# vainglorygame/analyzer

Measured on AMD Instinct MI355X. Metric: matches/sec rated (whole node), 3v3 TrueSkill, 1M-player roster, higher is better.
Workload: dtype fp32; 1 GPU; global_batch=10000000, seq_len=6, players=1000000, matches_per_gpu=10000000, team_size=3, parallelism=dp1, mode=exact, bench_config=2, skew=1, force_merge=False

## Files before the change

analyzer_amd/csrc/radix_sort.hip:

```cpp
#include <hip/hip_runtime.h>

#include <cstdlib>

#include "common.h"
#include "kernels.h"

namespace ana {

namespace {

#ifndef ANA_SORT_THREADS
#define ANA_SORT_THREADS 512
#endif
constexpr int kThreads = ANA_SORT_THREADS;
constexpr int kWaves = kThreads / 64;
constexpr int kItems = 16;
constexpr int kTile = kThreads * kItems;
constexpr int kRadix = 256;
constexpr int kRadixMax = 1024;

__device__ __forceinline__ int64_t xcd_tile(int64_t tiles) {
  const int64_t i = blockIdx.x, q = tiles >> 3, r = tiles & 7, x = i & 7;
  return x * q + (x < r ? x : r) + (i >> 3);
}

template <int NT>
__device__ __forceinline__ uint32_t ld32(const uint32_t* p) {
  if constexpr (NT >= 1) return __builtin_nontemporal_load(p);
  else return *p;
}
template <int NT>
__device__ __forceinline__ void st32(uint32_t* p, uint32_t v) {
  if constexpr (NT == 1) __builtin_nontemporal_store(v, p);
  else *p = v;
}

__device__ __forceinline__ uint32_t block_exclusive_scan(uint32_t x, uint32_t* wsum,
                                                         uint32_t* total) {
  const int lane = threadIdx.x & 63, wv = threadIdx.x >> 6;
  uint32_t inc = x;
#pragma unroll
  for (int off = 1; off < 64; off <<= 1) {
    const uint32_t y = __shfl_up(inc, off);
    if (lane >= off) inc += y;
  }
  if (lane == 63) wsum[wv] = inc;
  __syncthreads();
  uint32_t before = 0, all = 0;
#pragma unroll
  for (int w = 0; w < kWaves; ++w) {
    if (w < wv) before += wsum[w];
    all += wsum[w];
  }
  if (total) *total = all;
  __syncthreads();
  return before + inc - x;
}

template <int KS>
__device__ __forceinline__ void decode_tile_keys(const int32_t* __restrict__ rec, uint32_t kend,
                                                 int64_t base, int64_t n, uint32_t* lk, uint32_t knone) {
  constexpr int S = 2 * KS, R = S + 2;
  const uint32_t lo = (uint32_t)base;
  const uint32_t hi = (uint32_t)(base + kTile < n ? base + kTile : n);
  const uint32_t m_lo = lo / S, m_hi = (hi + S - 1) / S;
  for (uint32_t m = m_lo + threadIdx.x; m < m_hi; m += kThreads) {
    const int32_t* src = rec + (int64_t)m * R;
    int32_t r[R];
    if constexpr (R % 4 == 0) {
#pragma unroll
      for (int k = 0; k < R / 4; ++k) {
        const int4 v = reinterpret_cast<const int4*>(src)[k];
        r[4 * k] = v.x; r[4 * k + 1] = v.y; r[4 * k + 2] = v.z; r[4 * k + 3] = v.w;
      }
    } else {
#pragma unroll
      for (int k = 0; k < R; ++k) r[k] = src[k];
    }
    const bool rates = early_status<KS>(r, (int64_t)kend) == kRated;
    const uint32_t m0 = (uint32_t)r[S];
#pragma unroll
    for (int j = 0; j < S; ++j) {
      const uint32_t slot = m * S + j;
      const int pos = j < KS ? j : j - KS;
      const bool in_roster = pos < (j < KS ? meta_n0(m0) : meta_n1(m0));
      if (slot >= lo && slot < hi) lk[slot - lo] = rates && in_roster ? (uint32_t)r[j] : knone;
    }
  }
}

struct SchedInit {
  int32_t* deps = nullptr;
  uint32_t* ctrl = nullptr;
  int nz = 0;
  int32_t* epoch_bump = nullptr;
};

template <int KS, int RB = 8, int NT = 0>
__global__ void __launch_bounds__(kThreads)
radix_upsweep(const uint32_t* __restrict__ keys, const int32_t* __restrict__ rec, uint32_t kend,
              int64_t n, int shift, uint32_t* __restrict__ counts, int64_t tiles, SchedInit init = {},
              uint32_t knone = 0u) {
  constexpr int kR = 1 << RB;
  __shared__ uint32_t hist[kWaves][kR];
  __shared__ uint32_t lkeys[KS > 0 ? kTile : 1];
  const int tid = threadIdx.x, wv = tid >> 6;
  for (int i = tid; i < kWaves * kR; i += kThreads) (&hist[0][0])[i] = 0u;
  const int64_t tile = xcd_tile(tiles);
  const int64_t base = tile * kTile;
  if constexpr (KS > 0) {
    if (init.deps) {
      constexpr int S = 2 * KS;
      const int64_t hi = base + kTile < n ? base + kTile : n;
      for (int64_t m = (base + S - 1) / S + tid; m < (hi + S - 1) / S; m += kThreads) init.deps[m] = 0;
    }
    if (blockIdx.x == 0) {
      if (tid < init.nz) init.ctrl[tid] = 0u;
      if (tid == 0 && init.epoch_bump) init.epoch_bump[0] += 1;
    }
  }
  if constexpr (KS > 0) decode_tile_keys<KS>(rec, kend, base, n, lkeys, knone ? knone : kend);
  __syncthreads();
#pragma unroll
  for (int k = 0; k < kItems; ++k) {
    const int64_t idx = base + k * kThreads + tid;
    if (idx < n) {
      const uint32_t key = KS > 0 ? lkeys[k * kThreads + tid] : ld32<NT>(keys + idx);
      atomicAdd(&hist[wv][(key >> shift) & (kR - 1)], 1u);
    }
  }
  __syncthreads();
#pragma unroll
  for (int d = tid; d < kR; d += kThreads) {
    uint32_t c = 0;
#pragma unroll
    for (int w = 0; w < kWaves; ++w) c += hist[w][d];
    counts[(int64_t)d * tiles + tile] = c;
  }
}

template <int DPT>
__device__ __forceinline__ void digits_exclusive_scan(uint32_t (&v)[DPT], uint32_t* wsum,
                                                      uint32_t* total) {
  uint32_t s = 0;
#pragma unroll
  for (int j = 0; j < DPT; ++j) {
    const uint32_t x = v[j];
    v[j] = s;
    s += x;
  }
  const uint32_t before = block_exclusive_scan(s, wsum, total);
#pragma unroll
  for (int j = 0; j < DPT; ++j) v[j] += before;
}

__global__ void __launch_bounds__(kThreads)
radix_rowscan(uint32_t* __restrict__ counts, int64_t tiles, uint32_t* __restrict__ totals) {
  __shared__ uint32_t wsum[kWaves];
  constexpr int kPer = 4;
  uint32_t* row = counts + (int64_t)blockIdx.x * tiles;
  uint32_t carry = 0;
  for (int64_t start = 0; start < tiles; start += kThreads * kPer) {
    uint32_t v[kPer], s = 0;
#pragma unroll
    for (int q = 0; q < kPer; ++q) {
      const int64_t t = start + (int64_t)threadIdx.x * kPer + q;
      v[q] = t < tiles ? row[t] : 0u;
      s += v[q];
    }
    uint32_t all;
    uint32_t ex = carry + block_exclusive_scan(s, wsum, &all);
#pragma unroll
    for (int q = 0; q < kPer; ++q) {
      const int64_t t = start + (int64_t)threadIdx.x * kPer + q;
      if (t < tiles) row[t] = ex;
      ex += v[q];
    }
    carry += all;
  }
  if (threadIdx.x == 0) totals[blockIdx.x] = carry;
}

struct RunEnds {
  uint32_t kf, vf, kl, vl;
};
constexpr uint32_t kRunEmpty = 0xffffffffu;

template <int KS, bool LINK, int RB = 8, int NT = 0>
__global__ void __launch_bounds__(kThreads)
radix_downsweep(const uint32_t* __restrict__ kin, const uint32_t* __restrict__ vin,
                const int32_t* __restrict__ rec, uint32_t kend,
                uint32_t* __restrict__ kout, uint32_t* __restrict__ vout, int64_t n, int shift,
                const uint32_t* __restrict__ counts, const uint32_t* __restrict__ totals,
                int64_t tiles, int slots_per_match, uint32_t* __restrict__ link,
                uint32_t vlo = 0u, uint32_t vhi = 0xffffffffu, int bounds = 1,
                RunEnds* __restrict__ bnd = nullptr, int nd = 0, uint32_t knone = 0u) {
  constexpr int kR = 1 << RB;
  constexpr int DPT = kR >= kThreads ? kR / kThreads : 1;
  static_assert(kR % kThreads == 0 || kThreads % kR == 0, "radix and block must divide");
  __shared__ uint32_t skey[kTile];
  __shared__ uint32_t sval[kTile];
  __shared__ uint32_t wcnt[kWaves][kR];
  __shared__ uint32_t tstart[kR];
  __shared__ uint32_t gstart[kR];
  __shared__ uint32_t wsum[kWaves];
  const int tid = threadIdx.x, lane = tid & 63, wv = tid >> 6;
  const int64_t tile = xcd_tile(tiles);
  const int64_t base = tile * kTile;
  for (int i = tid; i < kWaves * kR; i += kThreads) (&wcnt[0][0])[i] = 0u;
  const bool local_ends = LINK && bnd != nullptr;
  if (!local_ends) {
    uint32_t v[DPT];
#pragma unroll
    for (int j = 0; j < DPT; ++j) v[j] = tid * DPT + j < kR ? totals[tid * DPT + j] : 0u;
    digits_exclusive_scan<DPT>(v, wsum, nullptr);
#pragma unroll
    for (int j = 0; j < DPT; ++j)
      if (tid * DPT + j < kR) gstart[tid * DPT + j] = v[j] + counts[(int64_t)(tid * DPT + j) * tiles + tile];
  }
  if constexpr (KS > 0)
    decode_tile_keys<KS>(rec, kend, base, n, sval, knone ? knone : kend);
  __syncthreads();

  const uint64_t lt_mask = (1ull << lane) - 1ull;
  uint32_t key[kItems], val[kItems], rank[kItems];
#pragma unroll
  for (int it = 0; it < kItems; ++it) {
    const int64_t idx = base + (int64_t)(wv * kItems + it) * 64 + lane;
    const bool valid = idx < n;
    if constexpr (KS > 0) key[it] = valid ? sval[(wv * kItems + it) * 64 + lane] : 0xffffffffu;
    else key[it] = valid ? ld32<NT>(kin + idx) : 0xffffffffu;
    if constexpr (KS == 0) val[it] = valid ? ld32<NT>(vin + idx) : 0u;
    else val[it] = (uint32_t)idx;
  }
#pragma unroll
  for (int it = 0; it < kItems; ++it) {
    const uint32_t d = (key[it] >> shift) & (kR - 1);
    uint64_t peers = ~0ull;
#pragma unroll
    for (int b = 0; b < RB; ++b) {
      const uint64_t bal = __ballot((d >> b) & 1u);
      peers &= ((d >> b) & 1u) ? bal : ~bal;
    }
    const uint32_t before = (uint32_t)__popcll(peers & lt_mask);
    const uint32_t run = wcnt[wv][d];
    rank[it] = run + before;
    if (before == (uint32_t)__popcll(peers) - 1u) wcnt[wv][d] = run + (uint32_t)__popcll(peers);
  }
  __syncthreads();
  {
    uint32_t v[DPT];
#pragma unroll
    for (int j = 0; j < DPT; ++j) {
      const int d = tid * DPT + j;
      uint32_t s = 0;
      if (d < kR) {
#pragma unroll
        for (int w = 0; w < kWaves; ++w) {
          const uint32_t c = wcnt[w][d];
          wcnt[w][d] = s;
          s += c;
        }
      }
      v[j] = s;
    }
    digits_exclusive_scan<DPT>(v, wsum, nullptr);
#pragma unroll
    for (int j = 0; j < DPT; ++j)
      if (tid * DPT + j < kR) tstart[tid * DPT + j] = v[j];
  }
  __syncthreads();
#pragma unroll
  for (int it = 0; it < kItems; ++it) {
    const uint32_t d = (key[it] >> shift) & (kR - 1);
    const uint32_t pos = tstart[d] + wcnt[wv][d] + rank[it];
    skey[pos] = key[it];
    sval[pos] = val[it];
  }
  __syncthreads();
  const int64_t nvalid = n - base < kTile ? n - base : kTile;
  if constexpr (LINK) {
    if (local_ends && bounds && tid < nd) {
      const uint32_t e = tid + 1 < kR ? tstart[tid + 1] : (uint32_t)kTile;
      if (tstart[tid] == e) bnd[tile * nd + tid].kf = kRunEmpty;
    }
  }
#pragma unroll
  for (int k = 0; k < kItems; ++k) {
    const int i = k * kThreads + tid;
    if (i < nvalid) {
      const uint32_t kk = skey[i];
      const uint32_t d = (kk >> shift) & (kR - 1);
      const int64_t o = local_ends ? 0 : (int64_t)gstart[d] + (i - (int64_t)tstart[d]);
      if constexpr (!LINK) {
        st32<NT>(kout + o, kk);
        st32<NT>(vout + o, sval[i]);
      } else {
        const int hi = d + 1 < (uint32_t)kR ? (int)tstart[d + 1] : kTile;
        const bool first = i == (int)tstart[d];
        const bool last = i + 1 == hi || i + 1 >= nvalid;
        const uint32_t v = sval[i];
        if (bounds && (first || last)) {
          if (local_ends) {
            if ((int)d < nd) {
              RunEnds* r = bnd + tile * nd + d;
              if (first) { r->kf = kk; r->vf = v; }
              if (last) { r->kl = kk; r->vl = v; }
            }
          } else {
            st32<NT>(kout + o, kk);
            st32<NT>(vout + o, v);
          }
        }
        if (kk < kend && v >= vlo && v < vhi) {
          uint32_t w = (!last && skey[i + 1] == kk) ? sval[i + 1] / (uint32_t)slots_per_match
                                                     : kNoMatch;
          if (!first && skey[i - 1] == kk) w |= kLinkHasPred;
          st32<NT>(link + v, w);
        }
      }
    }
  }
}

static bool local_runs() {
  const char* e = getenv("ANA_SCHED_RUNS");
  return !(e && atoi(e) == 0);
}

static int link_parts(int64_t n) {
  if (const char* e = getenv("ANA_LINK_PARTS")) {
    const int v = atoi(e);
    if (v >= 1) return v > 16 ? 16 : v;
  }
  const int64_t bytes = n * 4, part = 256ll << 20;
  return (int)((bytes + part - 1) / part);
}

template <int RB = 8>
__global__ void __launch_bounds__(kThreads)
sched_fixup(const uint32_t* __restrict__ kout, const uint32_t* __restrict__ vout, int64_t n,
            uint32_t kend, const uint32_t* __restrict__ counts, const uint32_t* __restrict__ totals,
            int64_t tiles, int slots_per_match, uint32_t* __restrict__ link) {
  constexpr int kR = 1 << RB;
  __shared__ uint32_t wsum[kWaves];
  const int d = blockIdx.y;
  const uint32_t tot = totals[d];
  if (tot == 0) return;
  uint32_t below = 0;
#pragma unroll
  for (int j = threadIdx.x; j < kR; j += kThreads) below += j < d ? totals[j] : 0u;
  uint32_t all = 0;
  const uint32_t before = block_exclusive_scan(below, wsum, &all);
  (void)before;
  const uint32_t dstart = all;
  const int64_t t = (int64_t)blockIdx.x * kThreads + threadIdx.x;
  if (t >= tiles) return;
  const uint32_t* row = counts + (int64_t)d * tiles;
  const uint32_t c0 = row[t];
  const uint32_t c1 = t + 1 < tiles ? row[t + 1] : tot;
  if (c1 == c0) return;
  const int64_t of = (int64_t)dstart + c0, ol = (int64_t)dstart + c1 - 1;
  const uint32_t kf = kout[of], kl = kout[ol];
  const bool pred = kf < kend && of > 0 && kout[of - 1] == kf;
  const bool succ = kl < kend && ol + 1 < n && kout[ol + 1] == kl;
  const uint32_t nxt = succ ? vout[ol + 1] / (uint32_t)slots_per_match : kNoMatch;
  if (of == ol) {
    if (kf < kend) link[vout[of]] = nxt | (pred ? kLinkHasPred : 0u);
    return;
  }
  if (pred) {
    const uint32_t v = vout[of];
    link[v] |= kLinkHasPred;
  }
  if (succ) {
    const uint32_t v = vout[ol];
    link[v] = (link[v] & ~kMatchMask) | nxt;
  }
}

constexpr int kRunsMaxDigits = 32;

__global__ void __launch_bounds__(kThreads)
sched_runs_last(const RunEnds* __restrict__ bnd, int64_t tiles, int nd, int32_t* __restrict__ seglast) {
  __shared__ int32_t wmax[kWaves];
  const int d = blockIdx.y;
  const int64_t t = (int64_t)blockIdx.x * kThreads + threadIdx.x;
  int32_t x = (t < tiles && bnd[t * nd + d].kf != kRunEmpty) ? (int32_t)t : -1;
#pragma unroll
  for (int off = 32; off >= 1; off >>= 1) x = max(x, __shfl_xor(x, off));
  if ((threadIdx.x & 63) == 0) wmax[threadIdx.x >> 6] = x;
  __syncthreads();
  if (threadIdx.x == 0) {
    int32_t m = wmax[0];
#pragma unroll
    for (int w = 1; w < kWaves; ++w) m = max(m, wmax[w]);
    seglast[(int64_t)d * gridDim.x + blockIdx.x] = m;
  }
}

__global__ void __launch_bounds__(kThreads)
sched_runs_fixup(const RunEnds* __restrict__ bnd, int64_t tiles, int nd, const int32_t* __restrict__ seglast,
                 uint32_t kend, int slots_per_match, uint32_t* __restrict__ link) {
  __shared__ int32_t wmax[kWaves];
  __shared__ int32_t carry_s;
  const int d = blockIdx.y, lane = threadIdx.x & 63, wv = threadIdx.x >> 6;
  const int64_t seg = blockIdx.x;
  if (wv == 0) {
    int32_t c = -1;
    for (int64_t q = lane; q < seg; q += 64) c = max(c, seglast[(int64_t)d * gridDim.x + q]);
#pragma unroll
    for (int off = 32; off >= 1; off >>= 1) c = max(c, __shfl_xor(c, off));
    if (lane == 0) carry_s = c;
  }
  const int64_t t = seg * kThreads + threadIdx.x;
  RunEnds me = {kRunEmpty, 0u, kRunEmpty, 0u};
  if (t < tiles) me = bnd[t * nd + d];
  const bool full = me.kf != kRunEmpty;
  int32_t x = full ? (int32_t)t : -1;
#pragma unroll
  for (int off = 1; off < 64; off <<= 1) {
    const int32_t y = __shfl_up(x, off);
    if (lane >= off) x = max(x, y);
  }
  if (lane == 63) wmax[wv] = x;
  __syncthreads();
  int32_t before = carry_s;
  for (int w = 0; w < wv; ++w) before = max(before, wmax[w]);
  int32_t ex = __shfl_up(x, 1);
  ex = lane == 0 ? -1 : ex;
  const int32_t pred = max(before, ex);
  if (!full || pred < 0 || me.kf >= kend) return;
  const RunEnds pr = bnd[(int64_t)pred * nd + d];
  if (pr.kl != me.kf) return;
  atomicOr(&link[me.vf], kLinkHasPred);
  atomicAnd(&link[pr.vl], ~kMatchMask | (me.vf / (uint32_t)slots_per_match));
}

constexpr int kChainLowBits = 12;
constexpr int kChainRB = 6;
constexpr uint32_t kChainEmpty = 0xffffffffu;
constexpr bool kChainDefault = true;

__device__ __forceinline__ void chain_sort_round(const uint32_t (&key)[kItems], const uint32_t (&val)[kItems],
                                                 int shift, uint32_t* skey, uint32_t* sval,
                                                 uint32_t (*wcnt)[1 << kChainRB], uint32_t* tstart,
                                                 uint32_t* wsum) {
  constexpr int kR = 1 << kChainRB;
  static_assert(kR <= kThreads, "one digit per thread in the scan");
  const int tid = threadIdx.x, lane = tid & 63, wv = tid >> 6;
  const uint64_t lt_mask = (1ull << lane) - 1ull;
  for (int i = tid; i < kWaves * kR; i += kThreads) (&wcnt[0][0])[i] = 0u;
  __syncthreads();
  uint32_t rank[kItems];
#pragma unroll
  for (int it = 0; it < kItems; ++it) {
    const uint32_t d = (key[it] >> shift) & (kR - 1);
    uint64_t peers = ~0ull;
#pragma unroll
    for (int b = 0; b < kChainRB; ++b) {
      const uint64_t bal = __ballot((d >> b) & 1u);
      peers &= ((d >> b) & 1u) ? bal : ~bal;
    }
    const uint32_t before = (uint32_t)__popcll(peers & lt_mask);
    const uint32_t run = wcnt[wv][d];
    rank[it] = run + before;
    if (before == (uint32_t)__popcll(peers) - 1u) wcnt[wv][d] = run + (uint32_t)__popcll(peers);
  }
  __syncthreads();
  {
    uint32_t v[1];
    uint32_t s = 0;
    if (tid < kR) {
#pragma unroll
      for (int w = 0; w < kWaves; ++w) {
        const uint32_t c = wcnt[w][tid];
        wcnt[w][tid] = s;
        s += c;
      }
    }
    v[0] = s;
    digits_exclusive_scan<1>(v, wsum, nullptr);
    if (tid < kR) tstart[tid] = v[0];
  }
  __syncthreads();
#pragma unroll
  for (int it = 0; it < kItems; ++it) {
    const uint32_t d = (key[it] >> shift) & (kR - 1);
    const uint32_t pos = tstart[d] + wcnt[wv][d] + rank[it];
    skey[pos] = key[it];
    sval[pos] = val[it];
  }
  __syncthreads();
}

template <int KS, int NT>
__global__ void __launch_bounds__(kThreads)
sched_chain(const uint32_t* __restrict__ kin, const uint32_t* __restrict__ vin,
            const int32_t* __restrict__ rec, uint32_t kend, int64_t n, int low,
            const uint32_t* __restrict__ totals, int slots_per_match, uint32_t* __restrict__ link,
            uint32_t vlo, uint32_t vhi, int64_t matches, SchedInit init) {
  constexpr int kR = 1 << kChainRB;
  __shared__ uint32_t skey[kTile];
  __shared__ uint32_t sval[kTile];
  __shared__ uint32_t last_seen[1 << kChainLowBits];
  __shared__ uint32_t wcnt[kWaves][kR];
  __shared__ uint32_t tstart[kR];
  __shared__ uint32_t wsum[kWaves];
  const int tid = threadIdx.x, lane = tid & 63, wv = tid >> 6;
  const uint32_t lmask = (1u << low) - 1u;
  for (int e = tid; e <= (int)lmask; e += kThreads) last_seen[e] = kChainEmpty;
  int64_t start = 0, cnt = n;
  if constexpr (KS > 0) {
    if (init.deps)
      for (int64_t m = tid; m < matches; m += kThreads) init.deps[m] = 0;
    if (tid < init.nz) init.ctrl[tid] = 0u;
    if (tid == 0 && init.epoch_bump) init.epoch_bump[0] += 1;
  } else {
    uint32_t below = 0;
    const uint32_t x = tid < (int)blockIdx.x ? totals[tid] : 0u;
    block_exclusive_scan(x, wsum, &below);
    start = below;
    cnt = totals[blockIdx.x];
  }
  for (int64_t base = 0; base < cnt; base += kTile) {
    const int64_t nvalid = cnt - base < kTile ? cnt - base : kTile;
    uint32_t key[kItems], val[kItems];
    if constexpr (KS > 0) {
      decode_tile_keys<KS>(rec, kend, base, n, sval, kend);
      __syncthreads();
    }
#pragma unroll
    for (int it = 0; it < kItems; ++it) {
      const int p = (wv * kItems + it) * 64 + lane;
      const bool valid = p < nvalid;
      const int64_t idx = start + base + p;
      if constexpr (KS > 0) {
        key[it] = valid ? sval[p] : 0xffffffffu;
        val[it] = (uint32_t)idx;
      } else {
        key[it] = valid ? ld32<NT>(kin + idx) : 0xffffffffu;
        val[it] = valid ? ld32<NT>(vin + idx) : 0u;
      }
    }
    chain_sort_round(key, val, 0, skey, sval, wcnt, tstart, wsum);
    if (low > kChainRB) {
#pragma unroll
      for (int it = 0; it < kItems; ++it) {
        const int p = (wv * kItems + it) * 64 + lane;
        key[it] = skey[p];
        val[it] = sval[p];
      }
      chain_sort_round(key, val, kChainRB, skey, sval, wcnt, tstart, wsum);
    }
    uint32_t is_last = 0u, has = 0u;
#pragma unroll 2
    for (int k = 0; k < kItems; ++k) {
      const int i = k * kThreads + tid;
      if (i < nvalid) {
        const uint32_t kk = skey[i];
        if (kk < kend) {
          const uint32_t v = sval[i];
          const bool next = i + 1 < nvalid && skey[i + 1] == kk;
          bool pred = i > 0 && skey[i - 1] == kk;
          if (!pred) {
            const uint32_t t = last_seen[kk & lmask];
            if (t != kChainEmpty) {
              pred = true;
              const uint32_t ts = t & kMatchMask;
              if (ts >= vlo && ts < vhi) link[ts] = v / (uint32_t)slots_per_match | (t & kLinkHasPred);
            }
          }
          if (next) {
            if (v >= vlo && v < vhi)
              link[v] = sval[i + 1] / (uint32_t)slots_per_match | (pred ? kLinkHasPred : 0u);
          } else {
            is_last |= 1u << k;
          }
          if (pred) has |= 1u << k;
        }
      }
    }
    __syncthreads();
#pragma unroll 2
    for (int k = 0; k < kItems; ++k) {
      const int i = k * kThreads + tid;
      if (is_last >> k & 1u) last_seen[skey[i] & lmask] = sval[i] | (has >> k & 1u ? kLinkHasPred : 0u);
    }
    __syncthreads();
  }
  __syncthreads();
  for (int e = tid; e <= (int)lmask; e += kThreads) {
    const uint32_t t = last_seen[e];
    if (t != kChainEmpty) {
      const uint32_t ts = t & kMatchMask;
      if (ts >= vlo && ts < vhi) link[ts] = kNoMatch | (t & kLinkHasPred);
    }
  }
}

}

size_t radix_sort_workspace_bytes(int64_t n) {
  const int64_t tiles = (n + kTile - 1) / kTile;
  return (size_t)(tiles * kRadixMax + kRadixMax) * 4;
}

int launch_radix_sort_pairs(uint32_t* keys, uint32_t* vals, uint32_t* keys_alt, uint32_t* vals_alt,
                            int64_t n, int bits, void* ws, int* result_in_alt, hipStream_t s) {
  *result_in_alt = 0;
  if (n <= 0) return 0;
  if (n > 0x7fffffffLL || bits < 1 || bits > 32) return (int)hipErrorInvalidValue;
  const int64_t tiles = (n + kTile - 1) / kTile;
  uint32_t* counts = static_cast<uint32_t*>(ws);
  uint32_t* totals = counts + tiles * kRadix;
  uint32_t *ki = keys, *vi = vals, *ko = keys_alt, *vo = vals_alt;
  for (int shift = 0; shift < bits; shift += 8) {
    hipLaunchKernelGGL(radix_upsweep<0>, dim3((unsigned)tiles), dim3(kThreads), 0, s, ki, nullptr,
                       0u, n, shift, counts, tiles);
    hipLaunchKernelGGL(radix_rowscan, dim3(kRadix), dim3(kThreads), 0, s, counts, tiles, totals);
    hipLaunchKernelGGL((radix_downsweep<0, false>), dim3((unsigned)tiles), dim3(kThreads), 0, s, ki,
                       vi, nullptr, 0u, ko, vo, n, shift, counts, totals, tiles, 1, nullptr);
    std::swap(ki, ko);
    std::swap(vi, vo);
    *result_in_alt ^= 1;
  }
  return (int)hipGetLastError();
}

template <int K, int RB, int NT>
static void sched_sort_k(const int32_t* rec, int64_t n, uint32_t kend, int bits, uint32_t* ka,
                         uint32_t* va, uint32_t* kb, uint32_t* vb, uint32_t* counts,
                         int64_t tiles, uint32_t* link, const SchedInit& init, bool chain,
                         hipStream_t s) {
  constexpr int S = 2 * K;
  constexpr int kR = 1 << RB;
  uint32_t* totals = counts + tiles * kR;
  const dim3 grid((unsigned)tiles), block(kThreads);
  const uint32_t *ki = nullptr, *vi = nullptr;
  uint32_t *ko = kb, *vo = vb;
  if (chain) {
    const int low = bits < kChainLowBits ? bits : kChainLowBits, top = bits - low;
    const int parts = link_parts(n);
    if (top > 0) {
      const uint32_t nb = ((kend - 1u) >> low) + 1u;
      const uint32_t knone = nb < (uint32_t)kR ? nb << low : kend;
      hipLaunchKernelGGL((radix_upsweep<K, RB, NT>), grid, block, 0, s, nullptr, rec, kend, n, low, counts, tiles,
                         init, knone);
      hipLaunchKernelGGL(radix_rowscan, dim3(kR), block, 0, s, counts, tiles, totals);
      hipLaunchKernelGGL((radix_downsweep<K, false, RB, NT>), grid, block, 0, s, nullptr, nullptr, rec, kend, ko,
                         vo, n, low, counts, totals, tiles, S, nullptr, 0u, 0xffffffffu, 1, nullptr, 0, knone);
      for (int q = 0; q < parts; ++q)
        hipLaunchKernelGGL((sched_chain<0, NT>), dim3(nb), block, 0, s, ko, vo, nullptr, kend, n, low,
                           totals, S, link, (uint32_t)(n * q / parts), (uint32_t)(n * (q + 1) / parts),
                           n / S, SchedInit{});
    } else {
      for (int q = 0; q < parts; ++q)
        hipLaunchKernelGGL((sched_chain<K, NT>), dim3(1), block, 0, s, nullptr, nullptr, rec, kend, n, low,
                           nullptr, S, link, (uint32_t)(n * q / parts), (uint32_t)(n * (q + 1) / parts),
                           n / S, q == 0 ? init : SchedInit{});
    }
    return;
  }
  for (int shift = 0; shift < bits; shift += RB) {
    const bool first = shift == 0, last = shift + RB >= bits;
    const int nd = bits - shift < RB ? 1 << (bits - shift) : kR;
    if (last && !first && nd <= kRunsMaxDigits && local_runs()) {
      RunEnds* bnd = reinterpret_cast<RunEnds*>(counts);
      const int64_t nseg = (tiles + kThreads - 1) / kThreads;
      int32_t* seglast = reinterpret_cast<int32_t*>(bnd + tiles * nd);
      const int parts = link_parts(n);
      for (int q = 0; q < parts; ++q)
        hipLaunchKernelGGL((radix_downsweep<0, true, RB, NT>), grid, block, 0, s, ki, vi, nullptr, kend, ko, vo,
                           n, shift, counts, totals, tiles, S, link, (uint32_t)(n * q / parts),
                           (uint32_t)(n * (q + 1) / parts), q == 0 ? 1 : 0, bnd, nd);
      const dim3 sgrid((unsigned)nseg, (unsigned)nd);
      hipLaunchKernelGGL(sched_runs_last, sgrid, block, 0, s, bnd, tiles, nd, seglast);
      hipLaunchKernelGGL(sched_runs_fixup, sgrid, block, 0, s, bnd, tiles, nd, seglast, kend, S, link);
      break;
    }
    if (first)
      hipLaunchKernelGGL((radix_upsweep<K, RB, NT>), grid, block, 0, s, nullptr, rec, kend, n, shift, counts, tiles,
                         init);
    else
      hipLaunchKernelGGL((radix_upsweep<0, RB, NT>), grid, block, 0, s, ki, nullptr, kend, n, shift, counts, tiles);
    hipLaunchKernelGGL(radix_rowscan, dim3(kR), block, 0, s, counts, tiles, totals);
    const int parts = last ? link_parts(n) : 1;
    if (first && last)
      for (int q = 0; q < parts; ++q)
        hipLaunchKernelGGL((radix_downsweep<K, true, RB, NT>), grid, block, 0, s, nullptr, nullptr, rec, kend, ko,
                           vo, n, shift, counts, totals, tiles, S, link, (uint32_t)(n * q / parts),
                           (uint32_t)(n * (q + 1) / parts), q == 0 ? 1 : 0);
    else if (first)
      hipLaunchKernelGGL((radix_downsweep<K, false, RB, NT>), grid, block, 0, s, nullptr, nullptr, rec, kend, ko,
                         vo, n, shift, counts, totals, tiles, S, nullptr);
    else if (last)
      for (int q = 0; q < parts; ++q)
        hipLaunchKernelGGL((radix_downsweep<0, true, RB, NT>), grid, block, 0, s, ki, vi, nullptr, kend, ko, vo,
                           n, shift, counts, totals, tiles, S, link, (uint32_t)(n * q / parts),
                           (uint32_t)(n * (q + 1) / parts), q == 0 ? 1 : 0);
    else
      hipLaunchKernelGGL((radix_downsweep<0, false, RB, NT>), grid, block, 0, s, ki, vi, nullptr, kend, ko, vo, n,
                         shift, counts, totals, tiles, S, nullptr);
    if (last)
      hipLaunchKernelGGL((sched_fixup<RB>), dim3((unsigned)((tiles + kThreads - 1) / kThreads), kR), block,
                         0, s, ko, vo, n, kend, counts, totals, tiles, S, link);
    ki = ko;
    vi = vo;
    ko = ko == kb ? ka : kb;
    vo = vo == vb ? va : vb;
  }
}

int launch_sched_sort(int K, const int32_t* rec, int64_t M, uint32_t num_players, uint32_t* ka,
                      uint32_t* va, uint32_t* kb, uint32_t* vb, void* ws, uint32_t* link,
                      hipStream_t s, int32_t* deps, uint32_t* ctrl, int nz, int32_t* epoch_bump,
                      int sort_nt) {
  const int64_t n = M * 2 * K;
  if (n <= 0) return 0;
  if (n > kMaxSlots) return (int)hipErrorInvalidValue;
  int bits = 1;
  while (bits < 32 && (1ull << bits) <= (uint64_t)num_players) ++bits;
  const int64_t tiles = (n + kTile - 1) / kTile;
  uint32_t* counts = static_cast<uint32_t*>(ws);
  SchedInit init;
  init.deps = deps;
  init.ctrl = ctrl;
  init.nz = ctrl ? nz : 0;
  init.epoch_bump = epoch_bump;
  const char* rb_e = getenv("ANA_SORT_RB");
  const char* nt_e = getenv("ANA_SORT_NT");
  const int rb_env = rb_e ? atoi(rb_e) : 8;
  const int nt = nt_e ? atoi(nt_e) : sort_nt >= 0 ? sort_nt : 0;
  const bool wide = bits <= 20 && rb_env == 10;
  const char* chain_e = getenv("ANA_SCHED_CHAIN");
  const int top = bits > kChainLowBits ? bits - kChainLowBits : 0;
  const bool chain_pays = (n >> top) <= 2 * kTile + n / 128;
  const bool chain = (chain_e ? atoi(chain_e) != 0 : kChainDefault && chain_pays) && bits <= 20 && !wide &&
                     local_runs();
  const bool known = with_team_size(K, [&](auto k) {
    constexpr int kK = decltype(k)::value;
    if (wide) sched_sort_k<kK, 10, 0>(rec, n, num_players, bits, ka, va, kb, vb, counts, tiles, link, init, chain, s);
    else if (nt == 1) sched_sort_k<kK, 8, 1>(rec, n, num_players, bits, ka, va, kb, vb, counts, tiles, link, init, chain, s);
    else if (nt == 2) sched_sort_k<kK, 8, 2>(rec, n, num_players, bits, ka, va, kb, vb, counts, tiles, link, init, chain, s);
    else sched_sort_k<kK, 8, 0>(rec, n, num_players, bits, ka, va, kb, vb, counts, tiles, link, init, chain, s);
  });
  return known ? (int)hipGetLastError() : (int)hipErrorInvalidValue;
}

}
```

Baseline: 1.578 billion matches/s.

## Write chain links in partitioned order then scatter back with an unpartition kernel

When the key space spans several buckets, the chain kernel no longer writes links by random match index across multiple partition passes. It instead writes each link into the partitioned key buffer in bucket order, buffering the current tile in shared memory and deferring tile tails. A new unpartition kernel then scatters those links back to original positions one tile at a time and uses vectorized stores where it can. The aim is to replace scattered global writes and the repeated link_parts launches with coalesced writes, at the cost of an extra kernel pass, extra reads of the partitioned buffers, and more shared memory per block.

New measurement: 1.680 billion matches/s, median of 6. 6.4% higher.

```diff
diff --git a/analyzer_amd/csrc/radix_sort.hip b/analyzer_amd/csrc/radix_sort.hip
--- a/analyzer_amd/csrc/radix_sort.hip
+++ b/analyzer_amd/csrc/radix_sort.hip
@@ -442,6 +442,7 @@
 constexpr uint32_t kChainEmpty = 0xffffffffu;
 constexpr bool kChainDefault = true;
 
+template <bool VALS = true>
 __device__ __forceinline__ void chain_sort_round(const uint32_t (&key)[kItems], const uint32_t (&val)[kItems],
                                                  int shift, uint32_t* skey, uint32_t* sval,
                                                  uint32_t (*wcnt)[1 << kChainRB], uint32_t* tstart,
@@ -489,20 +490,25 @@
     const uint32_t d = (key[it] >> shift) & (kR - 1);
     const uint32_t pos = tstart[d] + wcnt[wv][d] + rank[it];
     skey[pos] = key[it];
-    sval[pos] = val[it];
-  }
-  __syncthreads();
-}
-
-template <int KS, int NT>
+    if constexpr (VALS) sval[pos] = val[it];
+  }
+  __syncthreads();
+}
+
+constexpr uint32_t kLinkDeferred = 0xfffffffeu;
+constexpr uint32_t kLinkSkip = 0xffffffffu;
+
+template <int KS, int NT, bool LINES>
 __global__ void __launch_bounds__(kThreads)
-sched_chain(const uint32_t* __restrict__ kin, const uint32_t* __restrict__ vin,
+sched_chain(uint32_t* kio, const uint32_t* __restrict__ vin,
             const int32_t* __restrict__ rec, uint32_t kend, int64_t n, int low,
             const uint32_t* __restrict__ totals, int slots_per_match, uint32_t* __restrict__ link,
             uint32_t vlo, uint32_t vhi, int64_t matches, SchedInit init) {
   constexpr int kR = 1 << kChainRB;
+  static_assert(!LINES || KS == 0, "bucket positions need the partition");
   __shared__ uint32_t skey[kTile];
   __shared__ uint32_t sval[kTile];
+  __shared__ uint32_t lbuf[LINES ? kTile : 1];
   __shared__ uint32_t last_seen[1 << kChainLowBits];
   __shared__ uint32_t wcnt[kWaves][kR];
   __shared__ uint32_t tstart[kR];
@@ -523,6 +529,7 @@
     start = below;
     cnt = totals[blockIdx.x];
   }
+  const uint32_t kbase = LINES ? (uint32_t)blockIdx.x << low : 0u;
   for (int64_t base = 0; base < cnt; base += kTile) {
     const int64_t nvalid = cnt - base < kTile ? cnt - base : kTile;
     uint32_t key[kItems], val[kItems];
@@ -538,63 +545,201 @@
       if constexpr (KS > 0) {
         key[it] = valid ? sval[p] : 0xffffffffu;
         val[it] = (uint32_t)idx;
+      } else if constexpr (!LINES) {
+        key[it] = valid ? ld32<NT>(kio + idx) : 0xffffffffu;
+        val[it] = valid ? ld32<NT>(vin + idx) : 0u;
       } else {
-        key[it] = valid ? ld32<NT>(kin + idx) : 0xffffffffu;
-        val[it] = valid ? ld32<NT>(vin + idx) : 0u;
-      }
-    }
-    chain_sort_round(key, val, 0, skey, sval, wcnt, tstart, wsum);
+        key[it] = valid ? (ld32<NT>(kio + idx) & lmask) | (uint32_t)p << low : 0xffffffffu;
+        if (valid) sval[p] = ld32<NT>(vin + idx);
+      }
+    }
+    chain_sort_round<!LINES>(key, val, 0, skey, sval, wcnt, tstart, wsum);
     if (low > kChainRB) {
 #pragma unroll
       for (int it = 0; it < kItems; ++it) {
         const int p = (wv * kItems + it) * 64 + lane;
         key[it] = skey[p];
-        val[it] = sval[p];
-      }
-      chain_sort_round(key, val, kChainRB, skey, sval, wcnt, tstart, wsum);
+        if constexpr (!LINES) val[it] = sval[p];
+      }
+      chain_sort_round<!LINES>(key, val, kChainRB, skey, sval, wcnt, tstart, wsum);
     }
     uint32_t is_last = 0u, has = 0u;
+    if constexpr (!LINES) {
 #pragma unroll 2
-    for (int k = 0; k < kItems; ++k) {
-      const int i = k * kThreads + tid;
-      if (i < nvalid) {
-        const uint32_t kk = skey[i];
-        if (kk < kend) {
-          const uint32_t v = sval[i];
-          const bool next = i + 1 < nvalid && skey[i + 1] == kk;
-          bool pred = i > 0 && skey[i - 1] == kk;
-          if (!pred) {
-            const uint32_t t = last_seen[kk & lmask];
-            if (t != kChainEmpty) {
-              pred = true;
-              const uint32_t ts = t & kMatchMask;
-              if (ts >= vlo && ts < vhi) link[ts] = v / (uint32_t)slots_per_match | (t & kLinkHasPred);
+      for (int k = 0; k < kItems; ++k) {
+        const int i = k * kThreads + tid;
+        if (i < nvalid) {
+          const uint32_t kk = skey[i];
+          if (kk < kend) {
+            const uint32_t v = sval[i];
+            const bool next = i + 1 < nvalid && skey[i + 1] == kk;
+            bool pred = i > 0 && skey[i - 1] == kk;
+            if (!pred) {
+              const uint32_t t = last_seen[kk & lmask];
+              if (t != kChainEmpty) {
+                pred = true;
+                const uint32_t ts = t & kMatchMask;
+                if (ts >= vlo && ts < vhi) link[ts] = v / (uint32_t)slots_per_match | (t & kLinkHasPred);
+              }
             }
+            if (next) {
+              if (v >= vlo && v < vhi)
+                link[v] = sval[i + 1] / (uint32_t)slots_per_match | (pred ? kLinkHasPred : 0u);
+            } else {
+              is_last |= 1u << k;
+            }
+            if (pred) has |= 1u << k;
           }
-          if (next) {
-            if (v >= vlo && v < vhi)
-              link[v] = sval[i + 1] / (uint32_t)slots_per_match | (pred ? kLinkHasPred : 0u);
-          } else {
-            is_last |= 1u << k;
+        }
+      }
+      __syncthreads();
+#pragma unroll 2
+      for (int k = 0; k < kItems; ++k) {
+        const int i = k * kThreads + tid;
+        if (is_last >> k & 1u) last_seen[skey[i] & lmask] = sval[i] | (has >> k & 1u ? kLinkHasPred : 0u);
+      }
+    } else {
+      const int64_t prev = base - kTile;
+#pragma unroll 2
+      for (int k = 0; k < kItems; ++k) {
+        const int i = k * kThreads + tid;
+        if (i < nvalid) {
+          const uint32_t kl = skey[i] & lmask;
+          if ((kbase | kl) < kend) {
+            const bool next = i + 1 < nvalid && (skey[i + 1] & lmask) == kl;
+            bool pred = i > 0 && (skey[i - 1] & lmask) == kl;
+            if (!pred) {
+              const uint32_t t = last_seen[kl];
+              if (t != kChainEmpty) {
+                pred = true;
+                const int64_t tp = t & kMatchMask;
+                const uint32_t w = sval[skey[i] >> low] / (uint32_t)slots_per_match | (t & kLinkHasPred);
+                if (tp >= prev) lbuf[tp - prev] = w;
+                else kio[start + tp] = w;
+              }
+            }
+            if (!next) is_last |= 1u << k;
+            if (pred) has |= 1u << k;
           }
-          if (pred) has |= 1u << k;
         }
       }
+      __syncthreads();
+      if (base > 0) {
+#pragma unroll 2
+        for (int k = 0; k < kItems; ++k) {
+          const int j = k * kThreads + tid;
+          const uint32_t w = lbuf[j];
+          if (w != kLinkDeferred) st32<NT>(kio + start + prev + j, w);
+        }
+      }
+#pragma unroll 2
+      for (int k = 0; k < kItems; ++k) {
+        const int i = k * kThreads + tid;
+        if (is_last >> k & 1u) {
+          const uint32_t kk = skey[i];
+          last_seen[kk & lmask] = (uint32_t)(base + (kk >> low)) | (has >> k & 1u ? kLinkHasPred : 0u);
+        }
+      }
+      __syncthreads();
+#pragma unroll 2
+      for (int k = 0; k < kItems; ++k) {
+        const int i = k * kThreads + tid;
+        if (i < nvalid) {
+          const uint32_t kk = skey[i];
+          uint32_t w = kLinkSkip;
+          if ((kbase | (kk & lmask)) < kend)
+            w = is_last >> k & 1u ? kLinkDeferred
+                                  : sval[skey[i + 1] >> low] / (uint32_t)slots_per_match |
+                                        (has >> k & 1u ? kLinkHasPred : 0u);
+          lbuf[kk >> low] = w;
+        }
+      }
     }
     __syncthreads();
-#pragma unroll 2
-    for (int k = 0; k < kItems; ++k) {
-      const int i = k * kThreads + tid;
-      if (is_last >> k & 1u) last_seen[skey[i] & lmask] = sval[i] | (has >> k & 1u ? kLinkHasPred : 0u);
+  }
+  __syncthreads();
+  if constexpr (!LINES) {
+    for (int e = tid; e <= (int)lmask; e += kThreads) {
+      const uint32_t t = last_seen[e];
+      if (t != kChainEmpty) {
+        const uint32_t ts = t & kMatchMask;
+        if (ts >= vlo && ts < vhi) link[ts] = kNoMatch | (t & kLinkHasPred);
+      }
+    }
+  } else {
+    const int64_t lastb = cnt > 0 ? (cnt - 1) / kTile * kTile : 0;
+    for (int e = tid; e <= (int)lmask; e += kThreads) {
+      const uint32_t t = last_seen[e];
+      if (t != kChainEmpty) {
+        const int64_t tp = t & kMatchMask;
+        const uint32_t w = kNoMatch | (t & kLinkHasPred);
+        if (tp >= lastb) lbuf[tp - lastb] = w;
+        else kio[start + tp] = w;
+      }
     }
     __syncthreads();
-  }
-  __syncthreads();
-  for (int e = tid; e <= (int)lmask; e += kThreads) {
-    const uint32_t t = last_seen[e];
-    if (t != kChainEmpty) {
-      const uint32_t ts = t & kMatchMask;
-      if (ts >= vlo && ts < vhi) link[ts] = kNoMatch | (t & kLinkHasPred);
+    for (int64_t j = tid; j < cnt - lastb; j += kThreads) st32<NT>(kio + start + lastb + j, lbuf[j]);
+  }
+}
+
+template <int RB, int NT>
+__global__ void __launch_bounds__(kThreads)
+sched_unpartition(const uint32_t* __restrict__ lk, const uint32_t* __restrict__ vo, int64_t n,
+                  const uint32_t* __restrict__ counts, const uint32_t* __restrict__ totals,
+                  int64_t tiles, int nb, uint32_t* __restrict__ link) {
+  constexpr int kR = 1 << RB;
+  static_assert(kR <= kThreads, "one digit per thread");
+  __shared__ uint32_t out[kTile];
+  __shared__ uint32_t tstart[kR];
+  __shared__ uint32_t gstart[kR];
+  __shared__ uint32_t wsum[kWaves];
+  const int tid = threadIdx.x;
+  const int64_t tile = xcd_tile(tiles);
+  const int64_t base = tile * kTile;
+  const int64_t nvalid = n - base < kTile ? n - base : kTile;
+  uint32_t c0 = 0u, len = 0u;
+  if (tid < nb) {
+    c0 = counts[(int64_t)tid * tiles + tile];
+    len = (tile + 1 < tiles ? counts[(int64_t)tid * tiles + tile + 1] : totals[tid]) - c0;
+  }
+  uint32_t nchain = 0u;
+  const uint32_t g = block_exclusive_scan(tid < kR ? totals[tid] : 0u, wsum, nullptr);
+  const uint32_t ts = block_exclusive_scan(len, wsum, &nchain);
+  if (tid < kR) {
+    gstart[tid] = g + c0;
+    tstart[tid] = ts;
+  }
+#pragma unroll
+  for (int k = 0; k < kItems; ++k) out[k * kThreads + tid] = kLinkSkip;
+  __syncthreads();
+#pragma unroll 4
+  for (int k = 0; k < kItems; ++k) {
+    const uint32_t i = k * kThreads + tid;
+    if (i < nchain) {
+      uint32_t d = 0u;
+#pragma unroll
+      for (uint32_t step = kR >> 1; step > 0u; step >>= 1)
+        if (tstart[d + step] <= i) d += step;
+      const int64_t o = (int64_t)gstart[d] + (i - tstart[d]);
+      if (o < n) {
+        const uint32_t at = ld32<NT>(vo + o) - (uint32_t)base;
+        if (at < (uint32_t)kTile) out[at] = ld32<NT>(lk + o);
+      }
+    }
+  }
+  __syncthreads();
+#pragma unroll
+  for (int k = 0; k < kItems / 4; ++k) {
+    const int j = (k * kThreads + tid) * 4;
+    const uint4 w = *reinterpret_cast<const uint4*>(out + j);
+    const bool all = w.x != kLinkSkip && w.y != kLinkSkip && w.z != kLinkSkip && w.w != kLinkSkip;
+    if (j + 4 <= nvalid && all && (reinterpret_cast<uintptr_t>(link + base + j) & 15u) == 0u) {
+      *reinterpret_cast<uint4*>(link + base + j) = w;
+    } else {
+      if (j < nvalid && w.x != kLinkSkip) link[base + j] = w.x;
+      if (j + 1 < nvalid && w.y != kLinkSkip) link[base + j + 1] = w.y;
+      if (j + 2 < nvalid && w.z != kLinkSkip) link[base + j + 2] = w.z;
+      if (j + 3 < nvalid && w.w != kLinkSkip) link[base + j + 3] = w.w;
     }
   }
 }
@@ -641,7 +786,6 @@
   uint32_t *ko = kb, *vo = vb;
   if (chain) {
     const int low = bits < kChainLowBits ? bits : kChainLowBits, top = bits - low;
-    const int parts = link_parts(n);
     if (top > 0) {
       const uint32_t nb = ((kend - 1u) >> low) + 1u;
       const uint32_t knone = nb < (uint32_t)kR ? nb << low : kend;
@@ -650,13 +794,22 @@
       hipLaunchKernelGGL(radix_rowscan, dim3(kR), block, 0, s, counts, tiles, totals);
       hipLaunchKernelGGL((radix_downsweep<K, false, RB, NT>), grid, block, 0, s, nullptr, nullptr, rec, kend, ko,
                          vo, n, low, counts, totals, tiles, S, nullptr, 0u, 0xffffffffu, 1, nullptr, 0, knone);
+      if constexpr (NT != 0 && kR <= kThreads) {
+        hipLaunchKernelGGL((sched_chain<0, NT, true>), dim3(nb), block, 0, s, ko, vo, nullptr, kend, n, low,
+                           totals, S, nullptr, 0u, 0xffffffffu, n / S, SchedInit{});
+        hipLaunchKernelGGL((sched_unpartition<RB, NT>), grid, block, 0, s, ko, vo, n, counts, totals, tiles,
+                           (int)nb, link);
+      } else {
+        const int parts = link_parts(n);
+        for (int q = 0; q < parts; ++q)
+          hipLaunchKernelGGL((sched_chain<0, NT, false>), dim3(nb), block, 0, s, ko, vo, nullptr, kend, n, low,
+                             totals, S, link, (uint32_t)(n * q / parts), (uint32_t)(n * (q + 1) / parts),
+                             n / S, SchedInit{});
+      }
+    } else {
+      const int parts = link_parts(n);
       for (int q = 0; q < parts; ++q)
-        hipLaunchKernelGGL((sched_chain<0, NT>), dim3(nb), block, 0, s, ko, vo, nullptr, kend, n, low,
-                           totals, S, link, (uint32_t)(n * q / parts), (uint32_t)(n * (q + 1) / parts),
-                           n / S, SchedInit{});
-    } else {
-      for (int q = 0; q < parts; ++q)
-        hipLaunchKernelGGL((sched_chain<K, NT>), dim3(1), block, 0, s, nullptr, nullptr, rec, kend, n, low,
+        hipLaunchKernelGGL((sched_chain<K, NT, false>), dim3(1), block, 0, s, nullptr, nullptr, rec, kend, n, low,
                            nullptr, S, link, (uint32_t)(n * q / parts), (uint32_t)(n * (q + 1) / parts),
                            n / S, q == 0 ? init : SchedInit{});
     }
```
